# Jaroan/Contracts-MARL-AAM-Corridors

Measured on AMD Instinct MI355X. Metric: env-steps/sec (whole node) at 4096 envs x 10 agents, navigation_graph, higher is better.
Workload: dtype f64

## Files before the change

### contracts-marl-aam-corridors_amd/csrc/gmpe_kernel.h

```cpp
#pragma once
#include <hip/hip_runtime.h>
#include <math.h>
#include <stdio.h>
#include <stdlib.h>
#include <string.h>

#include <string>
#include <utility>
#include <vector>

#include "gmpe_device.h"

namespace gmpe {

enum { MODE_STEP = 0, MODE_RESET = 1 };
enum { SC_NAV = 0, SC_NAV_WALLS = 1, SC_JULY = 2, SC_ROT = 3, SC_TWO = 4, SC_THREE = 5, SC_COUNT = 6 };
__host__ __device__ constexpr bool sc_kinematic(int sc) { return sc >= SC_JULY; }
__host__ __device__ constexpr bool sc_rotfam(int sc) { return sc >= SC_ROT; }
__host__ __device__ constexpr bool sc_phasefam(int sc) { return sc == SC_TWO || sc == SC_THREE; }

struct KParams {
    gmpe_config c;
    DevState s;
    gmpe_outputs o;
// ... 107 lines not shown
template <int SC>
__device__ __forceinline__ void vel_of(double a2, double a3, double& vx, double& vy) {
    if (sc_kinematic(SC)) { double sn, cs; sincos(a2, &sn, &cs); vx = a3 * cs; vy = a3 * sn; }
    else { vx = a2; vy = a3; }
}

__device__ __forceinline__ bool wall_band_hit(const KParams& p, double px, double py, double size) {
    for (int w = 0; w < p.c.num_walls; ++w) {
        const gmpe_wall& wl = p.c.walls[w];
        const double band = 1.5 * size;
        const double perp = wl.orient == 0 ? py : px, prll = wl.orient == 0 ? px : py;
        if (wl.axis_pos - band <= perp && perp <= wl.axis_pos + band && wl.end0 - band <= prll && prll <= wl.end1 + band)
            return true;
    }
    return false;
}
__device__ __forceinline__ bool obstacle_collision_ego(const KParams& p, const Lds& l, int i) {
    const double* row = l.Dm + (size_t)i * p.E + p.A + p.L;
    for (int o = 0; o < p.O; ++o)
        if (row[o] < 2.0 * (p.c.entity_size + p.c.entity_size)) return true;
    return wall_band_hit(p, l.ex[i], l.ey[i], p.c.entity_size);
}

template <int SC>
__device__ __forceinline__ void decode_action(const gmpe_config& c, int idx, double& u0, double& u1) {
    if (!sc_kinematic(SC)) {
        if (c.n_actions == 5) {
            u0 = (idx == 1 ? 1.0 : 0.0) - (idx == 2 ? 1.0 : 0.0);
            u1 = (idx == 3 ? 1.0 : 0.0) - (idx == 4 ? 1.0 : 0.0);
        } else {
            const double d = 0.71;
            u0 = (idx == 1 ? -1.0 : idx == 5 ? 1.0 : (idx == 2 || idx == 8) ? -d : (idx == 4 || idx == 6) ? d : 0.0);
            u1 = (idx == 3 ? -1.0 : idx == 7 ? 1.0 : (idx == 2 || idx == 4) ? -d : (idx == 6 || idx == 8) ? d : 0.0);
        }
    } else {
        const int wi = idx / 5, ai = idx - wi * 5;
        u0 = wi == 0 ? c.ang_rate_opt[0] : wi == 1 ? c.ang_rate_opt[1] : wi == 2 ? c.ang_rate_opt[2] : wi == 3 ? c.ang_rate_opt[3] : c.ang_rate_opt[4];
        u1 = ai == 0 ? c.accel_opt[0] : ai == 1 ? c.accel_opt[1] : ai == 2 ? c.accel_opt[2] : ai == 3 ? c.accel_opt[3] : c.accel_opt[4];
    }
    u0 *= c.sensitivity; u1 *= c.sensitivity;
}

template <int AP, int SC>
__device__ __forceinline__ void write_obs(const KParams& p, const Lds& l, int i, double vx, double vy, int phase) {
    float* o = l.obs + (size_t)i * ((AP > 0 && (SC == SC_NAV || SC == SC_JULY)) ? (SC == SC_JULY ? 19 : 13) : p.D);
    const double px = l.ex[i], py = l.ey[i];
    const double gx = l.ex[(AP ? AP : p.A) + i] - px, gy = l.ey[(AP ? AP : p.A) + i] - py;
    o[0] = (float)px; o[1] = (float)py; o[2] = (float)vx; o[3] = (float)vy;
    o[4] = (float)gx; o[5] = (float)gy; o[6] = 0.0f; o[7] = (float)gx; o[8] = (float)gy;
    const double INF = __builtin_huge_val();
    int b1 = -1, b2 = -1; double d1 = INF, d2 = INF;
    const double* row = l.Dm + (size_t)i * ((AP > 0 && (SC == SC_NAV || SC == SC_JULY)) ? 2 * AP : p.E);
    if (AP) {
        double rv[AP ? AP : 1];
#pragma unroll
        for (int k = 0; k < AP; ++k) rv[k] = row[k < (AP ? AP : p.A) ? k : 0];
        __builtin_amdgcn_sched_barrier(0);
#pragma unroll
        for (int k = 0; k < AP; ++k) {
            const double d = (k < (AP ? AP : p.A) && k != i) ? rv[k] : INF;
            const bool lt1 = d < d1, lt2 = d < d2;
            d2 = lt1 ? d1 : (lt2 ? d : d2); b2 = lt1 ? b1 : (lt2 ? k : b2);
            d1 = lt1 ? d : d1; b1 = lt1 ? k : b1;
        }
    } else {
        for (int k = 0; k < (AP ? AP : p.A); ++k) {
            const double d = k != i ? row[k] : INF;
            const bool lt1 = d < d1, lt2 = d < d2;
            d2 = lt1 ? d1 : (lt2 ? d : d2); b2 = lt1 ? b1 : (lt2 ? k : b2);
            d1 = lt1 ? d : d1; b1 = lt1 ? k : b1;
        }
    }
    o[9] = b1 >= 0 ? (float)(l.ex[b1] - px) : 0.f; o[10] = b1 >= 0 ? (float)(l.ey[b1] - py) : 0.f;
    o[11] = b2 >= 0 ? (float)(l.ex[b2] - px) : 0.f; o[12] = b2 >= 0 ? (float)(l.ey[b2] - py) : 0.f;
    if (SC == SC_JULY) {
        o[13] = (float)(l.tube[T_ENTX] - px); o[14] = (float)(l.tube[T_ENTY] - py);
        o[15] = (float)(l.tube[T_EXX] - px); o[16] = (float)(l.tube[T_EXY] - py);
        o[17] = (float)l.tube[T_WIDTH]; o[18] = (float)phase;
    }
}

template <int AP, int SC>
__device__ __forceinline__ void write_obs_rot(const KParams& p, const Lds& l, int i, int phase) {
    float* o = l.obs + (size_t)i * p.D;
    const double px = l.ex[i], py = l.ey[i], th = l.s2[i];
    double sn, cs; sincos(th, &sn, &cs);
    const double INF = __builtin_huge_val();
    int b1 = -1, b2 = -1; double d1 = INF, d2 = INF;
    const double* row = l.Dm + (size_t)i * p.E;
    for (int k = 0; k < p.A; ++k) {
        bool skip = k == i;
        if (sc_phasefam(SC)) skip = skip || l.s_old[k] || (l.newf[k] && k < i);
        const double d = !skip ? row[k] : INF;
        const bool lt1 = d < d1, lt2 = d < d2;
        d2 = lt1 ? d1 : (lt2 ? d : d2); b2 = lt1 ? b1 : (lt2 ? k : b2);
        d1 = lt1 ? d : d1; b1 = lt1 ? k : b1;
    }
    double gx, gy;
    if (SC == SC_TWO) rot2(cs, sn, (double)(float)l.tube[T_EXX] - px, (double)(float)l.tube[T_EXY] - py, gx, gy);
    else rot2(cs, sn, l.ex[p.A + i] - px, l.ey[p.A + i] - py, gx, gy);
    double n1x = 0, n1y = 0, n2x = 0, n2y = 0;
    if (b1 >= 0) rot2(cs, sn, (double)(float)(l.ex[b1] - px), (double)(float)(l.ey[b1] - py), n1x, n1y);
    if (b2 >= 0) rot2(cs, sn, (double)(float)(l.ex[b2] - px), (double)(float)(l.ey[b2] - py), n2x, n2y);
    const double L = l.tube[T_L], hw = l.tube[T_HALFW];
    double s, yy; tube_sy(l.tube, px, py, s, yy);
    o[0] = (float)cs; o[1] = (float)sn; o[2] = (float)l.s3[i];
    o[3] = (float)gx; o[4] = (float)gy; o[5] = (float)n1x; o[6] = (float)n1y; o[7] = (float)n2x; o[8] = (float)n2y;
    o[9] = (float)clipd(s / L, -2.0, 2.0); o[10] = (float)clipd(yy / (hw + 1e-9), -2.0, 2.0);
    o[11] = (float)(exit_gate_distance(s, yy, L, hw) / (L + 1e-9));
    if (sc_phasefam(SC)) {
        double hs, hc; sincos(heading_error_signed(l.tube, th), &hs, &hc);
        o[12] = (float)hc; o[13] = (float)hs; o[14] = (float)phase;
    } else o[12] = (float)phase;
}

__device__ __forceinline__ double win_draw(const KParams& p, double* buf, int64_t& base, int W, int n, int i, int64_t k, int& err) {
    if (k >= base + W) {
        base = k;
        const int64_t kk = k + i;
        double val;
        if (p.s.tape) val = kk < p.s.tape_len ? p.s.tape[(size_t)n * p.s.tape_len + kk] : __builtin_nan("");
        else val = philox_uniform(p.c.seed, (uint32_t)(p.c.env_id_base + n), (uint64_t)kk);
        __builtin_amdgcn_fence(__ATOMIC_ACQUIRE, "wavefront");
        buf[i] = val;
        __builtin_amdgcn_fence(__ATOMIC_RELEASE, "wavefront");
        __builtin_amdgcn_wave_barrier();
        __builtin_amdgcn_fence(__ATOMIC_ACQUIRE, "wavefront");
    }
    double v = buf[(int)(k - base)];
    if (v != v) { err |= 1; v = 0.5; }
    return v;
}

__device__ __forceinline__ bool closer_than(double dx, double dy, double thr) {
    const double d2 = dx * dx + dy * dy, t2 = thr * thr;
    if (d2 < t2 * (1.0 - 1e-12)) return true;
    if (d2 > t2 * (1.0 + 1e-12)) return false;
    return sqrt(d2) < thr;
}
__device__ __forceinline__ double draw_raw(const KParams& p, int n, int64_t k) {
    if (p.s.tape) return k < p.s.tape_len ? p.s.tape[(size_t)n * p.s.tape_len + k] : 0.5;
    return philox_uniform(p.c.seed, (uint32_t)(p.c.env_id_base + n), (uint64_t)k);
}
__device__ __forceinline__ void wave_lds_sync() {
    __builtin_amdgcn_fence(__ATOMIC_RELEASE, "wavefront");
    __builtin_amdgcn_wave_barrier();
    __builtin_amdgcn_fence(__ATOMIC_ACQUIRE, "wavefront");
}
struct DrawBuf { const double* d; int64_t base; int nd; };
__device__ __forceinline__ double buf_get(const KParams& p, const DrawBuf& w, int n, int64_t k) {
    const int64_t o = k - w.base;
    return o < w.nd ? w.d[o] : draw_raw(p, n, k);
}
__device__ __forceinline__ void place_uniform(const KParams& p, const Lds& l, const DrawBuf& win, int n, int i, bool mine, unsigned long long emask, int M, int base, double thr,
                                              bool check_static, bool is_agent, int64_t& ctr, int& err) {
    const gmpe_config& c = p.c;
    const int A = p.A, O = p.O, o0 = p.A + p.L;
    const double ws = c.world_size, size = c.entity_size, lo = -ws / 2, hi = ws / 2;
    const int lane0 = emask ? __ffsll((long long)emask) - 1 : 0;
    double* cx = l.vox; double* cy = l.voy;
    unsigned long long* cm = reinterpret_cast<unsigned long long*>(l.vnx);
    int k = 0, tries = 0;
    while (__ballot(mine && k < M)) {
        if (mine && k < M) {
            const double px = 0.8 * (lo + (hi - lo) * buf_get(p, win, n, ctr + 2 * i));
            const double py = 0.8 * (lo + (hi - lo) * buf_get(p, win, n, ctr + 2 * i + 1));
            bool bad0 = false;
            if (check_static) {
                bad0 = wall_band_hit(p, px, py, size);
                for (int o = 0; o < O; ++o) bad0 = bad0 || closer_than(l.ex[o0 + o] - px, l.ey[o0 + o] - py, 2.0 * (size + size));
            }
            for (int q = 0; q < k; ++q) bad0 = bad0 || closer_than(l.ex[base + q] - px, l.ey[base + q] - py, thr);
            cx[i] = px; cy[i] = py;
            wave_lds_sync();
            unsigned long long cl = 0ull;
            for (int j = 0; j < i; ++j) if (closer_than(cx[j] - px, cy[j] - py, thr)) cl |= 1ull << j;
            cm[i] = cl;
            wave_lds_sync();
            const unsigned long long bad = (__ballot(bad0) & emask) >> lane0;
            unsigned long long acc = 0ull;
            int kk = k, t = tries, used = 0, slot = -1;
            for (int j = 0; j < A && kk < M; ++j) {
                const bool b = ((bad >> j) & 1ull) || (cm[j] & acc) != 0ull;
                used = j + 1;
                if (b && ++t < GMPE_MAX_TRIES) continue;
                if (b) err |= 2;
                if (j == i) slot = kk;
                acc |= 1ull << j; ++kk; t = 0;
            }
            wave_lds_sync();
            if (slot >= 0) {
                l.ex[base + slot] = px; l.ey[base + slot] = py;
                if (is_agent) { l.n2[slot] = 0.0; l.n3[slot] = 0.0; }
            }
            wave_lds_sync();
            ctr += 2 * used; k = kk; tries = t;
        }
    }
}

template <int SC, bool BATCH = false>
__device__ __forceinline__ void reset_world_coop(const KParams& p, const Lds& l, int n, int i, bool mine, unsigned long long emask, int64_t& ctr, int& err) {
    const gmpe_config& c = p.c;
    const double ws = c.world_size, size = c.entity_size;
    const int A = p.A, L = p.L, O = p.O;
    const int o0 = A + L;
    int64_t wbase = -(int64_t)A - 1;
    const int64_t ctr_in = ctr;
    const DrawBuf win = {reinterpret_cast<const double*>(l.M), ctr, BATCH ? (p.E * p.E + 3) / 4 * 2 : 0};
    const int lane0 = emask ? __ffsll((long long)emask) - 1 : 0;
#define WDRAW(k) (BATCH ? buf_get(p, win, n, (k)) : win_draw(p, l.serr, wbase, A, n, i, (k), err))
    if (sc_kinematic(SC)) {
        double entx = 0, enty = 0, exx = 0, exy = 0, sa = 0, ca = 1;
        if (mine) {
            (void)WDRAW(ctr++);
            const double a = 3 * size * 2.5, b = ws * 0.15;
            const double width = a > b ? a : b;
            const double angle = -M_PI / 2 + (M_PI / 2 - (-M_PI / 2)) * WDRAW(ctr++);
            double tl = ws * 0.8;
            if (sc_phasefam(SC)) tl += -ws * 0.3 + (ws * 0.1 - (-ws * 0.3)) * WDRAW(ctr++);
            ca = cos(angle); sa = sin(angle);
            const double be = tl / 4, bx = -tl / 4;
            entx = ca * 0 + sa * be; enty = -sa * 0 + ca * be;
            exx = ca * 0 + sa * bx; exy = -sa * 0 + ca * bx;
            const double dx = exx - entx, dy = exy - enty;
            const double Lt = sqrt(dx * dx + dy * dy) + 1e-9;
            const double ex = dx / Lt, ey = dy / Lt;
            if (i == 0) {
                double* t = l.tube;
                t[T_ANGLE] = angle; t[T_ENTX] = entx; t[T_ENTY] = enty; t[T_EXX] = exx; t[T_EXY] = exy;
                t[T_EX] = ex; t[T_EY] = ey; t[T_NX] = (double)(float)(-ey); t[T_NY] = (double)(float)ex;
                t[T_L] = Lt; t[T_HALFW] = width * 0.5; t[T_WIDTH] = width;
                for (int q = 0; q < GMPE_TUBE_STRIDE; ++q) p.s.tube[(size_t)n * GMPE_TUBE_STRIDE + q] = t[q];
            }
        }
        int k = 0, tries = 0;
        double mx = 0, my = 0;
        if constexpr (BATCH) while (__ballot(mine && k < A)) {
            if (mine && k < A) {
                const double u0 = buf_get(p, win, n, ctr + 2 * i), u1 = buf_get(p, win, n, ctr + 2 * i + 1);
                constexpr bool rot = sc_rotfam(SC);
                const double jf = rot ? 0.3 : 0.2;
                const double jx = jf * (-ws + (ws - (-ws)) * u0), jy = jf * (-ws + (ws - (-ws)) * u1);
                const double dfe = rot ? (ws + k) / 3 : (ws + k) / 5;
                const double px = entx + dfe * sa + jx, py = enty + dfe * ca + jy;
                bool bad_i = wall_band_hit(p, px, py, size);
                for (int o = 0; o < O; ++o) bad_i = bad_i || closer_than(l.ex[o0 + o] - px, l.ey[o0 + o] - py, 2.0 * (size + size));
                for (int q = 0; q < k; ++q) bad_i = bad_i || closer_than(l.ex[q] - px, l.ey[q] - py, c.sep_dist);
                const unsigned long long all = emask >> lane0;
                const unsigned long long good = ~((__ballot(bad_i) & emask) >> lane0) & all;
                const int jg = good ? __ffsll((long long)good) - 1 : A;
                const int jfo = GMPE_MAX_TRIES - 1 - tries;
                int js;
                if (jfo < A && jfo < jg) { js = jfo; err |= 2; }
                else if (jg < A) js = jg;
                else { tries += A; ctr += 2 * A; continue; }
                ctr += 2 * (js + 1);
                const double th = 0.0 + (2 * M_PI - 0.0) * buf_get(p, win, n, ctr); ++ctr;
                if (i == js) { l.ex[k] = px; l.ey[k] = py; l.n2[k] = th; l.n3[k] = c.v_min; }
                wave_lds_sync();
                ++k; tries = 0;
            }
        }
        else while (__ballot(mine && k < A)) {
            if (mine && k < A) {
                const double u0 = WDRAW(ctr), u1 = WDRAW(ctr + 1);
                ctr += 2;
                constexpr bool rot = sc_rotfam(SC);
                const double jf = rot ? 0.3 : 0.2;
                const double jx = jf * (-ws + (ws - (-ws)) * u0), jy = jf * (-ws + (ws - (-ws)) * u1);
                const double dfe = rot ? (ws + k) / 3 : (ws + k) / 5;
                const double px = entx + dfe * sa + jx, py = enty + dfe * ca + jy;
                bool bad_i = wall_band_hit(p, px, py, size);
                for (int o = i; o < O; o += A) bad_i = bad_i || norm2(l.ex[o0 + o] - px, l.ey[o0 + o] - py) < 2.0 * (size + size);
                bad_i = bad_i || (i < k && norm2(mx - px, my - py) < c.sep_dist);
                const bool bad = (__ballot(bad_i) & emask) != 0ull;
                if (bad && ++tries < GMPE_MAX_TRIES) continue;
                if (bad) err |= 2;
                const double th = 0.0 + (2 * M_PI - 0.0) * WDRAW(ctr++);
                if (i == k) { mx = px; my = py; l.ex[k] = px; l.ey[k] = py; l.n2[k] = th; l.n3[k] = c.v_min; }
                ++k; tries = 0;
            }
        }
        if (mine) {
            if (c.formation_type == GMPE_FORMATION_LINE) {
                const int div = L - 1;
                const double s0 = -ws / 2, e0 = ws / 2, ddx = e0 - s0, ddy = s0 - s0;
                for (int q = i; q < L; q += A) {
                    const double f = div > 0 ? (double)q / (double)div : (double)q;
                    double lx = f * ddx + s0, ly = f * ddy + s0;
                    if (L > 1 && q == L - 1) { lx = e0; ly = s0; }
                    bool hit = wall_band_hit(p, lx, ly, size);
                    for (int o = 0; o < O; ++o) hit = hit || norm2(l.ex[o0 + o] - lx, l.ey[o0 + o] - ly) < 2.0 * (size + size);
                    if (hit) err |= 2;
                    l.ex[A + q] = lx; l.ey[A + q] = ly;
                }
            } else if (c.formation_type == GMPE_FORMATION_CIRCLE) {
                const double cy = exy + ws / 5, radius = ws / 3, angle_step = 2 * M_PI / L;
                for (int q = i; q < L; q += A) {
                    const double ang = q * angle_step;
                    l.ex[A + q] = 0.0 + radius * cos(ang); l.ey[A + q] = cy + radius * sin(ang);
                }
            } else {
                const double rel = -ws / 3;
                const double rx = ca * 0.0 + sa * rel, ry = -sa * 0.0 + ca * rel;
                for (int q = i; q < L; q += A) { l.ex[A + q] = exx + rx; l.ey[A + q] = exy + ry; }
            }
        }
    } else if constexpr (BATCH) {
        place_uniform(p, l, win, n, i, mine, emask, O, o0, 2.0 * (size + size), false, false, ctr, err);
        place_uniform(p, l, win, n, i, mine, emask, A, 0, c.sep_dist, true, true, ctr, err);
        place_uniform(p, l, win, n, i, mine, emask, L, A, c.sep_dist, true, false, ctr, err);
        if (mine) for (int o = i; o < O; o += A) {
            p.s.obstacles[((size_t)n * O + o) * 2] = l.ex[o0 + o];
            p.s.obstacles[((size_t)n * O + o) * 2 + 1] = l.ey[o0 + o];
        }
    } else {
        const double lo = -ws / 2, hi = ws / 2;
        int k = 0, tries = 0;
        while (__ballot(mine && k < O)) {
            if (mine && k < O) {
                const double px = 0.8 * (lo + (hi - lo) * WDRAW(ctr));
                const double py = 0.8 * (lo + (hi - lo) * WDRAW(ctr + 1));
                ctr += 2;
                bool bad_i = false;
                for (int q = i; q < k; q += A) bad_i = bad_i || norm2(l.ex[o0 + q] - px, l.ey[o0 + q] - py) < 2.0 * (size + size);
                const bool bad = (__ballot(bad_i) & emask) != 0ull;
                if (bad && ++tries < GMPE_MAX_TRIES) continue;
                if (bad) err |= 2;
                if (k % A == i) { l.ex[o0 + k] = px; l.ey[o0 + k] = py; }
                ++k; tries = 0;
            }
        }
        k = 0; tries = 0;
        double mx = 0, my = 0;
        while (__ballot(mine && k < A)) {
            if (mine && k < A) {
                const double px = 0.8 * (lo + (hi - lo) * WDRAW(ctr));
                const double py = 0.8 * (lo + (hi - lo) * WDRAW(ctr + 1));
                ctr += 2;
                bool bad_i = wall_band_hit(p, px, py, size);
                for (int o = i; o < O; o += A) bad_i = bad_i || norm2(l.ex[o0 + o] - px, l.ey[o0 + o] - py) < 2.0 * (size + size);
                bad_i = bad_i || (i < k && norm2(mx - px, my - py) < c.sep_dist);
                const bool bad = (__ballot(bad_i) & emask) != 0ull;
                if (bad && ++tries < GMPE_MAX_TRIES) continue;
                if (bad) err |= 2;
                if (i == k) { mx = px; my = py; l.ex[k] = px; l.ey[k] = py; l.n2[k] = 0.0; l.n3[k] = 0.0; }
                ++k; tries = 0;
            }
        }
        k = 0; tries = 0;
        while (__ballot(mine && k < L)) {
            if (mine && k < L) {
                const double px = 0.8 * (lo + (hi - lo) * WDRAW(ctr));
                const double py = 0.8 * (lo + (hi - lo) * WDRAW(ctr + 1));
                ctr += 2;
                bool bad_i = wall_band_hit(p, px, py, size);
                for (int o = i; o < O; o += A) bad_i = bad_i || norm2(l.ex[o0 + o] - px, l.ey[o0 + o] - py) < 2.0 * (size + size);
                for (int r = i; r < k; r += A) bad_i = bad_i || norm2(l.ex[A + r] - px, l.ey[A + r] - py) < c.sep_dist;
                const bool bad = (__ballot(bad_i) & emask) != 0ull;
                if (bad && ++tries < GMPE_MAX_TRIES) continue;
                if (bad) err |= 2;
                if (k % A == i) { l.ex[A + k] = px; l.ey[A + k] = py; }
                ++k; tries = 0;
            }
        }
        if (mine) for (int o = i; o < O; o += A) {
            p.s.obstacles[((size_t)n * O + o) * 2] = l.ex[o0 + o];
            p.s.obstacles[((size_t)n * O + o) * 2 + 1] = l.ey[o0 + o];
        }
    }
    if (mine) for (int q = i; q < L; q += A) {
        p.s.landmarks[((size_t)n * L + q) * 2] = l.ex[A + q];
        p.s.landmarks[((size_t)n * L + q) * 2 + 1] = l.ey[A + q];
    }
    if (BATCH && mine && p.s.tape && ctr > ctr_in && ctr > p.s.tape_len) err |= 1;
}
#undef WDRAW


template <int BLOCK, int U, int CA>
__device__ __forceinline__ void distance_trip(const KParams& p, const Lds& l, int q0, int total, int W, int dv, bool even, bool only_reset) {
    const int A = CA ? CA : p.A, E = CA ? 2 * CA : p.E, AE = A * E, EE4 = (E * E + 3) / 4 * 4;
    double ds[U]; int gs[U], rs[U], cs[U];
#pragma unroll
    for (int u = 0; u < U; ++u) {
        const int q = q0 + u * BLOCK;
        const bool live = q < total;
        const int qq = live ? q : 0;
        const int g = fdiv(qq, W, p.m_W), w = qq - g * W;
        const int a = fdiv(w, dv, p.m_Sx), b = w - a * dv;
        int r, cc;
        if (even) { const bool up = b >= a; r = up ? a : E - 1 - a; cc = up ? b + 1 : E - a + b; }
        else { int c0 = a + 1 + b; c0 = c0 >= E ? c0 - E : c0; r = a < c0 ? a : c0; cc = a < c0 ? c0 : a; }
        const double dx = l.ex[g * E + r] - l.ex[g * E + cc], dy = l.ey[g * E + r] - l.ey[g * E + cc];
        ds[u] = (GMPE_ABL(p) & 16) ? dx * dx + dy * dy : sqrt(dx * dx + dy * dy);
        gs[u] = (live && !(only_reset && !l.flags[g * 4 + 0])) ? g : -1; rs[u] = r; cs[u] = cc;
    }
#pragma unroll
    for (int u = 0; u < U; ++u) {
        if (gs[u] < 0) continue;
        const int r = rs[u], cc = cs[u];
        float* Mg = l.M + (size_t)gs[u] * EE4;
        const float df = (float)ds[u];
        Mg[r * E + cc] = df; Mg[cc * E + r] = df;
        if (r < A) {
            double* Dg = l.Dm + (size_t)gs[u] * AE;
            Dg[r * E + cc] = ds[u];
            if (cc < A) Dg[cc * E + r] = ds[u];
        }
    }
}
template <int BLOCK, int CA>
__device__ __forceinline__ void distance_pass(const KParams& p, const Lds& l, int G, int tid, bool only_reset) {
    const int A = CA ? CA : p.A, E = CA ? 2 * CA : p.E, AE = A * E, EE4 = (E * E + 3) / 4 * 4;
    const int W = E * (E - 1) / 2;
    const bool even = (E & 1) == 0;
    const int dv = even ? E - 1 : (E - 1) / 2;
    const int total = G * W;
    const int wave_base = tid & ~63;
    for (int base = 0; base + wave_base < total; base += 5 * BLOCK) {
        const int left = total - (base + wave_base);
        const int nu = (left + BLOCK - 1) / BLOCK;
        const int q0 = base + tid;
        if (nu >= 5) distance_trip<BLOCK, 5, CA>(p, l, q0, total, W, dv, even, only_reset);
        else if (nu == 4) distance_trip<BLOCK, 4, CA>(p, l, q0, total, W, dv, even, only_reset);
        else if (nu == 3) distance_trip<BLOCK, 3, CA>(p, l, q0, total, W, dv, even, only_reset);
        else if (nu == 2) distance_trip<BLOCK, 2, CA>(p, l, q0, total, W, dv, even, only_reset);
        else distance_trip<BLOCK, 1, CA>(p, l, q0, total, W, dv, even, only_reset);
    }
    for (int q = tid; q < G * E; q += BLOCK) {
        const int g = fdiv(q, E, p.m_E), r = q - g * E;
        if (only_reset && !l.flags[g * 4 + 0]) continue;
        l.M[(size_t)g * EE4 + r * E + r] = 0.0f;
        if (r < A) l.Dm[(size_t)g * AE + r * E + r] = 0.0;
    }
}

#define GMPE_NSTAMPS 32
#ifdef GMPE_STAMPS
#define STAMP(k) do { if (tid == 0 && p.stamps) p.stamps[(size_t)blockIdx.x * GMPE_NSTAMPS + (k)] = __builtin_readcyclecounter(); } while (0)
#define STAMP_T(k, t) do { if (tid == (t) && p.stamps) p.stamps[(size_t)blockIdx.x * GMPE_NSTAMPS + (k)] = __builtin_readcyclecounter(); } while (0)
#else
#define STAMP(k) do { } while (0)
#define STAMP_T(k, t) do { } while (0)
#endif
template <int BLOCK, int CA, bool FORCES>
__device__ __forceinline__ void distance_force_pass(const KParams& p, const Lds& l, int G, int Gv, int tid, bool only_reset, bool statics) {
    constexpr int A = CA, E = 2 * CA, AE = A * E, EE4 = (E * E + 3) / 4 * 4, NP = A * (A - 1) / 2, NL = A * A;
    const gmpe_config& c = p.c;
    double* Fx = l.F2; double* Fy = Fx + (size_t)G * A * A;
    const int n1 = Gv * NP, n2 = n1 + Gv * NL, total = n2 + (statics ? Gv * NP : 0);
    const int wave_base = tid & ~63;
    for (int base = 0; base + wave_base < total; base += 3 * BLOCK) {
        double ds[3], dxs[3], dys[3]; int gs[3], rs[3], cs[3];
#pragma unroll
        for (int u = 0; u < 3; ++u) {
            const int q = base + u * BLOCK + tid;
            const bool live = q < total;
            const int qq = live ? q : 0;
            int g, r, cc;
            if (qq < n1) { g = qq / NP; const int pk = l.ptab[qq - g * NP]; r = pk >> 8; cc = pk & 255; }
            else if (qq < n2) { const int t = qq - n1; g = t / NL; const int w = t - g * NL; r = w / A; cc = A + (w - r * A); }
            else { const int t = qq - n2; g = t / NP; const int pk = l.ptab[t - g * NP]; r = A + (pk >> 8); cc = A + (pk & 255); }
            const double dx = l.ex[g * E + r] - l.ex[g * E + cc], dy = l.ey[g * E + r] - l.ey[g * E + cc];
            dxs[u] = dx; dys[u] = dy; ds[u] = sqrt(dx * dx + dy * dy);
            gs[u] = (live && !(only_reset && !l.flags[g * 4 + 0])) ? g : -1; rs[u] = r; cs[u] = cc;
        }
#pragma unroll
        for (int u = 0; u < 3; ++u) {
            if (gs[u] < 0) continue;
            const int r = rs[u], cc = cs[u];
            float* Mg = l.M + (size_t)gs[u] * EE4;
            const float df = (float)ds[u];
            Mg[r * E + cc] = df; Mg[cc * E + r] = df;
            if (r < A) {
                double* Dg = l.Dm + (size_t)gs[u] * AE;
                Dg[r * E + cc] = ds[u];
                if (cc < A) Dg[cc * E + r] = ds[u];
            }
        }
#pragma unroll
        for (int u = 0; u < 3; ++u) {
            if (!FORCES) break;
            if (base + u * BLOCK + wave_base >= n1) continue;
            if (gs[u] < 0 || cs[u] >= A) continue;
            const double dmin = c.contact_family ? c.agent_size + c.agent_size : c.sep_dist;
            const double pen = logaddexp0(-(ds[u] - dmin) / c.contact_margin) * c.contact_margin;
            const int slot = gs[u] * A * A + rs[u] * A + cs[u];
            Fx[slot] = c.contact_force * dxs[u] / ds[u] * pen; Fy[slot] = c.contact_force * dys[u] / ds[u] * pen;
        }
    }
    for (int q = tid; q < G * E; q += BLOCK) {
        const int g = q / E, r = q - g * E;
        if (only_reset && !l.flags[g * 4 + 0]) continue;
        if (r >= A && !statics) continue;
        l.M[(size_t)g * EE4 + r * E + r] = 0.0f;
        if (r < A) l.Dm[(size_t)g * AE + r * E + r] = 0.0;
    }
}

#define SWEEP(var, n) _Pragma("unroll") for (int var = 0; var < (AP ? AP : (n)); ++var)
template <int BLOCK, int AP, int SC, int FL>
__device__ __forceinline__ void stream_graph_fn(const KParams& p, const gmpe_outputs& o, const Lds& l, const int Gv, const int n0, const int tid,
                                                const int t0, const int nthr, const bool do_mask, const int any_mask) {
    constexpr bool CT = AP > 0 && SC != SC_NAV_WALLS;
    const int A = CT ? AP : p.A, L = CT ? AP : p.L, E = CT ? 2 * AP : p.E, EE = E * E, EE4 = (EE + 3) / 4 * 4;
    const int abl = FL ? 0 : GMPE_ABL(p);
    const bool nt = FL == 1 ? false : p.nt != 0;
    if (do_mask && any_mask && !(abl & 4)) {
        for (int q = tid; q < Gv * EE; q += BLOCK) {
            const int gg = fdiv(q, EE, p.m_EE), rc = q - gg * EE;
            if (!l.flags[gg * 4 + 2]) continue;
            const int r = fdiv(rc, E, p.m_E), cc = rc - r * E;
            if (l.moff[gg * E + r] | l.moff[gg * E + cc]) l.M[(size_t)gg * EE4 + rc] = 0.0f;
        }
    }
    if (do_mask) __syncthreads();
    

    if (o.adj && !(abl & 1)) {
        const bool vec = (EE & 3) == 0;
        if (o.adj_compact) {
            float* dst = o.adj + (size_t)n0 * EE;
            if (vec) {
                const int nq = EE / 4;
                for (int q = t0; q < Gv * nq; q += nthr) {
                    const int gg = fdiv(q, nq, p.m_nq), m = q - gg * nq;
                    if (l.flags[gg * 4 + 3]) reinterpret_cast<float4*>(dst)[q] = reinterpret_cast<const float4*>(l.M + (size_t)gg * EE4)[m];
                }
            } else for (int q = t0; q < Gv * EE; q += nthr) { const int gg = fdiv(q, EE, p.m_EE); if (l.flags[gg * 4 + 3]) dst[q] = l.M[(size_t)gg * EE4 + (q - gg * EE)]; }
        } else {
            float* dst = o.adj + (size_t)n0 * A * EE;
#ifdef GMPE_NTORDER_KNOB
            if (vec && nt && p.ablate != 200) {
#else
            if (vec && nt) {
#endif
                const int nq = EE / 4, per = A * nq;
                for (int gg = 0; gg < Gv; ++gg) {
                    if (!l.flags[gg * 4 + 3]) continue;
                    const float4* M4 = reinterpret_cast<const float4*>(l.M + (size_t)gg * EE4);
                    float4* d4 = reinterpret_cast<float4*>(dst) + (size_t)gg * per;
                    for (int q = t0; q < per; q += nthr) {
                        const int a = fdiv(q, nq, p.m_nq), m = q - a * nq;
                        nt_store4(&d4[q], M4[m]);
                    }
                }
            } else if (vec) {
                const int nq = EE / 4;
                for (int q = t0; q < Gv * nq; q += nthr) {
                    const int gg = fdiv(q, nq, p.m_nq), m = q - gg * nq;
                    if (!l.flags[gg * 4 + 3]) continue;
                    const float4 val = reinterpret_cast<const float4*>(l.M + (size_t)gg * EE4)[m];
                    float4* d4 = reinterpret_cast<float4*>(dst) + (size_t)gg * A * nq + m;
                    SWEEP(a, A) { if (!AP || a < A) { if (nt) nt_store4(&d4[(size_t)a * nq], val); else d4[(size_t)a * nq] = val; } }
                }
            } else {
                const int AEE = A * EE;
                for (int q = t0; q < Gv * AEE; q += nthr) {
                    const int gg = q / AEE, rem = q - gg * AEE, rc = rem % EE;
                    if (l.flags[gg * 4 + 3]) dst[q] = l.M[(size_t)gg * EE4 + rc];
                }
            }
        }
    }
    
    STAMP_T(16, 64); STAMP_T(19, 192);
    if (o.entity_table) {
        const int W = p.TW;
        double* dst = o.entity_table + (size_t)n0 * W;
        for (int q = t0; q < Gv * W; q += nthr) {
            const int gg = fdiv(q, W, p.m_TW), w = q - gg * W;
            if (!l.flags[gg * 4 + 3]) continue;
            double val;
            const int wm = W - (E + 31) / 32;
            if (w < 2 * E) val = w < E ? l.ex[gg * E + w] : l.ey[gg * E + (w - E)];
            else if (w >= wm) {
                unsigned bits = 0;
                const int k0 = (w - wm) * 32;
                for (int b = 0; b < 32 && k0 + b < E; ++b) bits |= (l.moff[gg * E + k0 + b] ? 1u : 0u) << b;
                val = (double)bits;
            }
            else if (SC == SC_TWO && w >= wm - 2) val = l.tube[gg * GMPE_TUBE_STRIDE + (w == wm - 2 ? T_EXX : T_EXY)];
            else {
                const int r = w - 2 * E, blk = fdiv(r, A, p.m_A), a = gg * A + (r - blk * A);
                val = blk == 0 ? l.vox[a] : blk == 1 ? l.voy[a] : blk == 2 ? l.vnx[a] : blk == 3 ? l.vny[a] : blk == 4 ? l.cn[a] : l.sn[a];
            }
            dst[q] = val;
        }
    }
    if (sc_rotfam(SC) && o.node_obs && !(abl & 2) && p.c.graph_feat_type != 1) {
// ... 541 lines not shown
                            double hx, hy; sincos(v.s2[i], &hy, &hx);
                            int front = -1, back = -1; double fproj = 0, bproj = 0;
                            for (int k = 0; k < A; ++k) {
                                if (k == i) continue;
                                const double pj = (v.ex[k] - px) * hx + (v.ey[k] - py) * hy;
                                if (pj > 0) { if (front < 0 || pj < fproj) { front = k; fproj = pj; } }
                                else { if (back < 0 || pj > bproj) { back = k; bproj = pj; } }
                            }
                            if (front >= 0) { const double df = row[front] - c.sep_dist; serr += df < 0 ? fabs(df) : 0; }
                            if (back >= 0) { const double df = row[back] - c.sep_dist; serr += df < 0 ? fabs(df) : 0; }
                            if (serr > 0) sv += 1;
                            rew -= serr * c.formation_rew;
                            rew -= exit_gate_distance(ts, ty, Lt, hw);
                            if (rotinv) {
                                const double tdx = v.tube[T_EXX] - v.tube[T_ENTX], tdy = v.tube[T_EXY] - v.tube[T_ENTY];
                                const double tlen = sqrt(tdx * tdx + tdy * tdy);
                                const double proj = (px - v.tube[T_ENTX]) * (tdx / tlen) + (py - v.tube[T_ENTY]) * (tdy / tlen);
                                const double gain = c.goal_rew / (c.world_size * 0.8 * 10);
                                const double dproj = proj - pproj;
                                rew += gain * (dproj > -0.05 ? dproj : -0.05);
                                pproj = (double)(float)proj;
                            } else rew -= herr * c.formation_rew * 0.1;
                            sic += 1;
                        } else if (rotinv && cp == 2 && phase_reached == 0) cp = 0;
                        else if (cp == 2 && !two) {
                            if (dgoal < c.goal_thresh) { if (me_new) rew += c.goal_rew * 5; }
                            else rew -= dgoal;
                        }
                        if (phase_reached == 1 && cp == 0) conf += 1;
                        if (cp > phase_reached) phase_reached = cp;
                        if (cp < prev_phase) rew -= c.collision_rew;
                        if (cp < phase_reached) rew -= c.collision_rew;
                        prev_phase = cp;
                        if (in_tube_rect(ts, ty, Lt, hw) && cp != 1 && !(three && in_exit_gate(ts, ty, Lt, hw, 0.02))) rew -= c.collision_rew;
                        if (ts > Lt && phase_reached < 1) rew -= c.goal_rew;
                    } else {
                        if (dgoal < c.goal_thresh) { if (me_new) rew += c.goal_rew * 5; }
                        else rew -= dgoal;
                    }
                    rew = clipd(rew, -4 * c.collision_rew, c.goal_rew * 5);
                    if (!rotfam) rew = clipd(rew, c.min_reward, c.max_reward);
                    v.serr[i] = two ? 0.0 : serr; v.rew[i] = rew;

                    STAMP(15);
                    v.dtg_o[i] = dtg; v.trq_o[i] = trq;
                    int nearest = 0; double dmin = INF;
                    SWEEP(q, L) { const bool ok = !AP || q < L; const double d = ok ? row[A + (ok ? q : 0)] : INF; const bool lt = d < dmin; dmin = lt ? d : dmin; nearest = lt ? q : nearest; }
                    const double thr = c.goal_thresh;
                    const int tnow = (int)((double)cur_step * c.dt);
                    if (dmin < thr && (nearest != greached && greached != -1)) { greached = nearest; dleft = (int)dmin; }
                    if (dmin < thr && trq == -1) { trq = tnow; dtg = (int)p_dist; dleft = (int)dmin; greached = nearest; }
                    if (trq == -1) { dtg = (int)p_dist; dleft = (int)dmin; }
                    if (dmin > thr && trq != -1) { dtg = (int)p_dist; trq = tnow; dleft = (int)dmin; }
                    if (dmin < thr && nearest == greached) { dleft = (int)dmin; greached = nearest; }
                    v.dtg_n[i] = dtg; v.trq_n[i] = trq;
                    v.sv_n[i] = sv; v.sv_o[i] = sv - (serr > 0 ? 1 : 0);
                }
                if (block_sync) __syncthreads();
                else {
                    __builtin_amdgcn_fence(__ATOMIC_RELEASE, "wavefront");
                    __builtin_amdgcn_wave_barrier();
                    __builtin_amdgcn_fence(__ATOMIC_ACQUIRE, "wavefront");
                }
                STAMP(6);

                if (ag) {
                    double rsum = 0;
                    if (c.collaborative) for (int a = 0; a < A; ++a) rsum += v.rew[a];
                    if (out.reward) out.reward[na] = (float)(c.collaborative ? rsum : rew);
                    if (out.done) out.done[na] = done ? 1 : 0;
                    if (ROLL) {
                        if (p.masks) p.masks[(size_t)slot * p.st_mask + na] = done ? 0.0f : 1.0f;
                        if (p.active) p.active[(size_t)slot * p.st_mask + na] = (done && !all_done) ? 0.0f : 1.0f;
                    }
                    if (out.info) {
                        double sd = 0, st = 0, sdd = 0, stt = 0; int ssv = 0;
                        SWEEP(a, A) {
                            const bool ok = !AP || a < A;
                            const int ac = ok ? a : 0;
                            const bool nw = ac <= i;
                            const int dn = v.dtg_n[ac], d_o = v.dtg_o[ac], tn = v.trq_n[ac], to = v.trq_o[ac], svn = v.sv_n[ac], svo = v.sv_o[ac];
                            const double dd = ok ? (double)(nw ? dn : d_o) : 0.0, tt = ok ? (double)(nw ? tn : to) : 0.0;
                            sd += dd; st += tt; sdd += dd * dd; stt += tt * tt;
                            ssv += ok ? (nw ? svn : svo) : 0;
                        }
                        double dsp = dsp0;
                        if (july || rotfam) for (int a = 0; a <= i; ++a) dsp += v.serr[a];
                        const double dm = sd / A, tm = st / A;
                        const double dvn = (double)A * sdd - sd * sd, tvn = (double)A * stt - st * st;
                        const double ds = sqrt(dvn) / A, ts = sqrt(tvn) / A;
                        float* o = out.info + na * GMPE_INFO_KEYS;
                        o[0] = (float)rew; o[1] = (float)dleft; o[2] = (float)trq; o[3] = (float)nac; o[4] = (float)noc;
                        o[5] = (float)dm; o[6] = (float)ds; o[7] = (float)(dm / (ds + 0.0001)); o[8] = (float)dtg;
                        o[9] = (float)trq; o[10] = (float)tm; o[11] = (float)ts; o[12] = (float)(tm / (ts + 0.0001));
                        o[13] = (float)((double)conf / c.episode_length);
                        o[14] = (float)(dsp / (ssv != 0 ? (double)ssv : 1.0));
                        o[15] = (float)((double)sv / (sic != 0 ? sic : 1));
                        o[16] = (float)gmt;
                        o[17] = (float)phase_reached;
                    }
                    if (ROLL && !all_done && kk + 1 < K) {
                        int* ci = l.cnt + (size_t)(g * A + i) * 9;
                        ci[0] = trq; ci[1] = dtg; ci[2] = dleft; ci[3] = greached; ci[4] = nac; ci[5] = noc; ci[6] = sv; ci[7] = sic; ci[8] = conf;
                        if (rotinv) l.cntd[(size_t)(g * A + i) * 2 + 1] = pproj;
                        if (i == 0) {
                            double dsp = dsp0;
                            if (july || rotfam) for (int a = 0; a < A; ++a) dsp += v.serr[a];
                            l.cntd[(size_t)G * A * 2 + g] = dsp;
                        }
                    } else if (!all_done) {
                        if (i == 0) {
                            double dsp = dsp0;
                            if (july || rotfam) for (int a = 0; a < A; ++a) dsp += v.serr[a];
                            p.s.delta_spacing[n] = dsp;
                            p.s.rng_ctr[n] = ctr0 + v.flags[1];
                            p.s.current_step[n] = cur_step;
                        }
                        p.s.x[na] = v.ex[i]; p.s.y[na] = v.ey[i]; p.s.s2[na] = v.n2[i]; p.s.s3[na] = v.n3[i];
                        p.s.status[na] = (uint8_t)(v.s_old[i] || v.newf[i]);
                        p.s.prev_phase[na] = prev_phase; p.s.phase_reached[na] = phase_reached; p.s.cooldown[na] = cooldown;
                        p.s.goal_tracker[na] = v.gt[i]; p.s.p_dist[na] = p_dist; p.s.time[na] = tim;
                        p.s.times_required[na] = trq; p.s.dists_to_goal[na] = dtg; p.s.dist_left[na] = dleft;
                        p.s.goal_reached[na] = greached; p.s.n_agent_coll[na] = nac; p.s.n_obst_coll[na] = noc;
                        p.s.spacing_viol[na] = sv; p.s.steps_in_corr[na] = sic; p.s.conformance[na] = conf;
                        if (rotinv) p.s.prev_proj[na] = pproj;
                    }
                }
                STAMP(7);
                if (spec && !ROLL) {
                    __builtin_amdgcn_fence(__ATOMIC_RELEASE, "wavefront");
                    __builtin_amdgcn_wave_barrier();
                    __builtin_amdgcn_fence(__ATOMIC_ACQUIRE, "wavefront");
                    if (out.obs) {
                        float* dst = out.obs + (size_t)n0 * A * D;
                        const int AD = A * D;
                        for (int q = tid; q < Gv * AD; q += 64) { const int gg = fdiv(q, AD, p.m_AD); if (l.flags[gg * 4 + 3]) dst[q] = l.obs[(size_t)gg * AD4 + (q - gg * AD)]; }
                    }
                    if (out.agent_id) for (int q = tid; q < Gv * A; q += 64) { const int gg = fdiv(q, A, p.m_A); if (l.flags[gg * 4 + 3]) out.agent_id[(size_t)n0 * A + q] = q - gg * A; }
                }
            }
            else {
                STAMP_T(9, 64); STAMP_T(17, 192);
                stream_graph_fn<BLOCK, AP, SC, FL>(p, out, l, Gv, n0, tid, tid - 64, BLOCK - 64, false, any_mask);
                STAMP_T(10, 64); STAMP_T(18, 192);
            }
            __syncthreads();
        }
        {
            if (any_reset) {
                const bool mine = ag && v.flags[0];
                if (tid < 64) {
                    int64_t ctr = ctr0 + ((mine && step) ? v.flags[1] : 0);
                    STAMP(20);
                    reset_world_coop<SC, BATCHK>(p, v, n, i, mine, emask, ctr, err);
                    STAMP(21);
                    if (mine && i == 0) {
                        if (ROLL) reinterpret_cast<long long*>(l.cntd + (size_t)G * A * 2 + G)[g] = ctr;
                        p.s.rng_ctr[n] = ctr;
                        p.s.current_step[n] = 0;
                        p.s.delta_spacing[n] = 0.0;
                        v.flags[2] = 0;
                    }
                }
                __syncthreads();
                if (mine) {
                    v.s2[i] = v.n2[i]; v.s3[i] = v.n3[i];
                    double vx, vy; vel_of<SC>(v.n2[i], v.n3[i], vx, vy);
                    v.vox[i] = v.vnx[i] = vx; v.voy[i] = v.vny[i] = vy;
                    v.s_old[i] = 0; v.newf[i] = 0; v.gt[i] = -1; v.moff[i] = 0; v.moff[A + i] = 0;
                    int prevA = prev_phase, ph = 0;
                    if (july) ph = phase_eval(v.tube, v.ex[i], v.ey[i], prev_phase, prevA);
                    prev_phase = prevA;
                    if (rotfam) { ph = phase_eval_rot<PV>(v.tube, v.ex[i], v.ey[i], prev_phase, 0); double sn_, cn_; sincos(v.n2[i], &sn_, &cn_); v.cn[i] = cn_; v.sn[i] = sn_; p.s.prev_proj[na] = 0.0; }
                    const double dx = v.ex[i] - v.ex[A + i], dy = v.ey[i] - v.ey[A + i];
                    gmt = c.max_speed > 0 ? sqrt(dx * dx + dy * dy) / c.max_speed : 0.0;
                    p.s.x[na] = v.ex[i]; p.s.y[na] = v.ey[i]; p.s.s2[na] = v.n2[i]; p.s.s3[na] = v.n3[i];
                    p.s.status[na] = 0; p.s.prev_phase[na] = prev_phase; p.s.phase_reached[na] = 0; p.s.cooldown[na] = 0;
                    p.s.goal_tracker[na] = -1; p.s.p_dist[na] = 0.0; p.s.time[na] = 0.0;
                    p.s.times_required[na] = -1; p.s.dists_to_goal[na] = -1; p.s.dist_left[na] = -1;
                    p.s.goal_reached[na] = -1; p.s.n_agent_coll[na] = 0; p.s.n_obst_coll[na] = 0;
                    p.s.spacing_viol[na] = 0; p.s.steps_in_corr[na] = 0; p.s.conformance[na] = 0;
                    p.s.goal_min_time[na] = gmt;
                    ph1 = ph;
                }
                STAMP(22);
                __syncthreads();
                if constexpr (FUSE_OK) {
                    if (FUSE) distance_force_pass<BLOCK, AP, !kin>(p, l, G, Gv, tid, true, true);
                    else distance_pass<BLOCK, (CT ? AP : 0)>(p, l, Gv, tid, true);
                } else distance_pass<BLOCK, (CT ? AP : 0)>(p, l, Gv, tid, true);
                __syncthreads();
                STAMP(23);
                if (mine) { if (rotfam) write_obs_rot<AP, SC>(p, v, i, ph1); else write_obs<AP, SC>(p, v, i, v.vox[i], v.voy[i], ph1); }
                any_mask = 0;
                for (int gg = 0; gg < Gv; ++gg) any_mask |= l.flags[gg * 4 + 2];
            }
            STAMP(8);
        }
        if (ROLL && !early) {
            __builtin_amdgcn_fence(__ATOMIC_RELEASE, "workgroup");
            __syncthreads();
        }
        if (!early) stream_graph_fn<BLOCK, AP, SC, FL>(p, out, l, Gv, n0, tid, tid, BLOCK, true, any_mask);
        STAMP(11);
        if (!spec || ROLL) {
            if (out.obs) {
                float* dst = out.obs + (size_t)n0 * A * D;
                const int AD = A * D;
                for (int q = tid; q < Gv * AD; q += BLOCK) { const int gg = fdiv(q, AD, p.m_AD); if (l.flags[gg * 4 + 3]) dst[q] = l.obs[(size_t)gg * AD4 + (q - gg * AD)]; }
            }
            if (out.agent_id) for (int q = tid; q < Gv * A; q += BLOCK) { const int gg = fdiv(q, A, p.m_A); if (l.flags[gg * 4 + 3]) out.agent_id[(size_t)n0 * A + q] = q - gg * A; }
        }
        if (ROLL && kk + 1 < K) {
            if (!early) __builtin_amdgcn_fence(__ATOMIC_RELEASE, "workgroup");
            if (!spec || !early) __syncthreads();
            if (ag) {
                if (all_done) {
                    phase_reached = 0; cooldown = 0; p_dist = 0.0; tim = 0.0; cur_step = 0;
                    ctr0 = reinterpret_cast<const long long*>(l.cntd + (size_t)G * A * 2 + G)[g];
                    int* ci = l.cnt + (size_t)(g * A + i) * 9;
                    ci[0] = -1; ci[1] = -1; ci[2] = -1; ci[3] = -1; ci[4] = 0; ci[5] = 0; ci[6] = 0; ci[7] = 0; ci[8] = 0;
                    l.cntd[(size_t)(g * A + i) * 2] = gmt; l.cntd[(size_t)(g * A + i) * 2 + 1] = 0.0;
                    if (i == 0) l.cntd[(size_t)G * A * 2 + g] = 0.0;
                } else {
                    v.s2[i] = v.n2[i]; v.s3[i] = v.n3[i];
                    v.s_old[i] = (v.s_old[i] || v.newf[i]) ? 1 : 0;
                    ctr0 += ndraw;
                }
                const int na_ = c.n_actions;
                act_idx = act_next < 0 ? 0 : (act_next >= na_ ? na_ - 1 : act_next);
            }
            for (int q = tid; q < G * E; q += BLOCK) l.moff[q] = 0;
            if (tid < G) {
                const bool active = n0 + tid < p.env_hi;
                l.flags[tid * 4 + 0] = 0; l.flags[tid * 4 + 1] = 0; l.flags[tid * 4 + 2] = 0; l.flags[tid * 4 + 3] = active;
            }
            slot = slot + 1 == p.num_slots ? 0 : slot + 1;
            __syncthreads();
        }
    } while (ROLL && ++kk < K);
    if (ag && err) atomicOr(&p.s.error_flags[n], err);
    STAMP(12);
}


struct EnvKernel {
    const void* fn;
    int threads;
    bool fuse;
};
template <int SC> EnvKernel env_kernel(int block, int ap, int fl, int G);

}
```

Baseline: 212.0 million.

## Specialize batched reset placement with compile-time agent count and unrolled masks

Adds a compile-time-size path for uniform placement during batched resets. It keeps the candidate-rejection loop in registers with unrolled squared-distance masks and a branchless greedy acceptance scan, and ping-pongs two LDS buffers to drop one wave barrier per round. It also assumes obstacles are zero and landmarks equal the agent count, and shrinks the draw window to match. The aim is to cut reset latency in the navigation scenario. The risk is divergence from the generic path if those assumptions do not hold, plus extra register pressure.

```diff
diff --git a/contracts-marl-aam-corridors_amd/csrc/gmpe_kernel.h b/contracts-marl-aam-corridors_amd/csrc/gmpe_kernel.h
--- a/contracts-marl-aam-corridors_amd/csrc/gmpe_kernel.h
+++ b/contracts-marl-aam-corridors_amd/csrc/gmpe_kernel.h
@@ -283,12 +283,111 @@
     const int64_t o = k - w.base;
     return o < w.nd ? w.d[o] : draw_raw(p, n, k);
 }
+#define GMPE_NSTAMPS 32
+#ifdef GMPE_STAMPS
+#define PSTAMP(k, val) do { if (threadIdx.x == 0 && p.stamps) p.stamps[(size_t)blockIdx.x * GMPE_NSTAMPS + (k)] = (val); } while (0)
+#else
+#define PSTAMP(k, val) do { } while (0)
+#endif
+template <int CA = 0>
 __device__ __forceinline__ void place_uniform(const KParams& p, const Lds& l, const DrawBuf& win, int n, int i, bool mine, unsigned long long emask, int M, int base, double thr,
                                               bool check_static, bool is_agent, int64_t& ctr, int& err) {
     const gmpe_config& c = p.c;
     const int A = p.A, O = p.O, o0 = p.A + p.L;
     const double ws = c.world_size, size = c.entity_size, lo = -ws / 2, hi = ws / 2;
     const int lane0 = emask ? __ffsll((long long)emask) - 1 : 0;
+    if constexpr (CA > 0) {
+        static_assert(CA <= 16, "a sweep's mask is half of a 32-bit word");
+        constexpr int N1 = CA > 1 ? CA : 1;
+        const int row = (int)(l.s3 - l.s2);
+        const double* ex = l.ex + base; const double* ey = l.ey + base;
+        const double t2 = thr * thr, t2lo = t2 * (1.0 - 1e-12), t2hi = t2 * (1.0 + 1e-12);
+        int k = 0, tries = 0, set = 0, rounds = 0;
+        while (__ballot(mine && k < CA)) {
+            if (mine && k < CA) {
+                if (is_agent && k == 0) PSTAMP(24, __builtin_readcyclecounter());
+                const int so = set ? row : 0;
+                double* cx = l.s2 + so; double* cy = l.vox + so; unsigned* cm = reinterpret_cast<unsigned*>(l.vnx + so);
+                const int64_t o = ctr + 2 * i - win.base;
+                double u0 = 0.0, u1 = 0.0;
+                if (o + 1 < win.nd) { u0 = win.d[o]; u1 = win.d[o + 1]; }
+                else {
+#pragma unroll 1
+                    for (int d = 0; d < 2; ++d) { u0 = u1; u1 = draw_raw(p, n, ctr + 2 * i + d); }
+                }
+                const double px = 0.8 * (lo + (hi - lo) * u0), py = 0.8 * (lo + (hi - lo) * u1);
+                cx[i] = px; cy[i] = py;
+                wave_lds_sync();
+                unsigned ltm = 0u, ngm = 0u;
+                {
+                    double qx[N1], qy[N1];
+#pragma unroll
+                    for (int q = 0; q < CA; ++q) { qx[q] = ex[q]; qy[q] = ey[q]; }
+                    __builtin_amdgcn_sched_barrier(0);
+#pragma unroll
+                    for (int q = 0; q < CA; ++q) {
+                        const double dx = qx[q] - px, dy = qy[q] - py, d2 = dx * dx + dy * dy;
+                        ltm |= d2 < t2lo ? 1u << q : 0u;
+                        ngm |= !(d2 > t2hi) ? 1u << q : 0u;
+                    }
+                }
+                const unsigned km = (1u << k) - 1u, im = (1u << i) - 1u;
+                unsigned hit = ltm & km, band = ngm & ~ltm & km;
+                ltm = 0u; ngm = 0u;
+                {
+                    double jx[N1], jy[N1];
+#pragma unroll
+                    for (int j = 0; j < CA; ++j) { jx[j] = cx[j]; jy[j] = cy[j]; }
+                    __builtin_amdgcn_sched_barrier(0);
+#pragma unroll
+                    for (int j = 0; j < CA; ++j) {
+                        const double dx = jx[j] - px, dy = jy[j] - py, d2 = dx * dx + dy * dy;
+                        ltm |= d2 < t2lo ? 1u << j : 0u;
+                        ngm |= !(d2 > t2hi) ? 1u << j : 0u;
+                    }
+                }
+                unsigned cl = ltm & im;
+                band |= (ngm & ~ltm & im) << 16;
+                while (band) {
+                    const int b = __ffs((int)band) - 1, q = b & 15; band &= band - 1u;
+                    if (closer_than((b < 16 ? ex : cx)[q] - px, (b < 16 ? ey : cy)[q] - py, thr)) { if (b < 16) hit |= 1u << q; else cl |= 1u << q; }
+                }
+                const bool bad0 = hit != 0u;
+                cm[i] = cl;
+                wave_lds_sync();
+                const unsigned bad = (unsigned)((__ballot(bad0) & emask) >> lane0);
+                unsigned cmr[N1];
+#pragma unroll
+                for (int j = 0; j < CA; ++j) cmr[j] = cm[j];
+                __builtin_amdgcn_sched_barrier(0);
+                unsigned acc = 0u;
+                int kk = k, t = tries, used = 0;
+#pragma unroll
+                for (int j = 0; j < CA; ++j) {
+                    const unsigned live = (unsigned)(kk - CA) >> 31;
+                    const unsigned b = ((bad >> j) & 1u) | min(cmr[j] & acc, 1u);
+                    const unsigned forced = b & ((unsigned)(GMPE_MAX_TRIES - 2 - t) >> 31);
+                    const unsigned take = live & ((b ^ 1u) | forced);
+                    used += (int)live;
+                    err |= (int)((live & forced) << 1);
+                    t = (t + (int)live) & ((int)take - 1);
+                    acc |= take << j;
+                    kk += (int)take;
+                }
+                const int slot = ((acc >> i) & 1u) ? k + __popc(acc & ((1u << i) - 1u)) : -1;
+                if (slot >= 0) {
+                    l.ex[base + slot] = px; l.ey[base + slot] = py;
+                    if (is_agent) { l.n2[slot] = 0.0; l.n3[slot] = 0.0; }
+                }
+                if (is_agent && k == 0) PSTAMP(25, __builtin_readcyclecounter());
+                ctr += 2 * used; k = kk; tries = t; set ^= 1;
+            }
+            ++rounds;
+        }
+        wave_lds_sync();
+        PSTAMP(is_agent ? 26 : 27, (unsigned long long)rounds);
+        return;
+    }
     double* cx = l.vox; double* cy = l.voy;
     unsigned long long* cm = reinterpret_cast<unsigned long long*>(l.vnx);
     int k = 0, tries = 0;
@@ -330,7 +429,7 @@
     }
 }
 
-template <int SC, bool BATCH = false>
+template <int SC, bool BATCH = false, int CA = 0>
 __device__ __forceinline__ void reset_world_coop(const KParams& p, const Lds& l, int n, int i, bool mine, unsigned long long emask, int64_t& ctr, int& err) {
     const gmpe_config& c = p.c;
     const double ws = c.world_size, size = c.entity_size;
@@ -338,7 +437,7 @@
     const int o0 = A + L;
     int64_t wbase = -(int64_t)A - 1;
     const int64_t ctr_in = ctr;
-    const DrawBuf win = {reinterpret_cast<const double*>(l.M), ctr, BATCH ? (p.E * p.E + 3) / 4 * 2 : 0};
+    const DrawBuf win = {reinterpret_cast<const double*>(l.M), ctr, BATCH ? ((CA ? 4 * CA * CA : p.E * p.E) + 3) / 4 * 2 : 0};
     const int lane0 = emask ? __ffsll((long long)emask) - 1 : 0;
 #define WDRAW(k) (BATCH ? buf_get(p, win, n, (k)) : win_draw(p, l.serr, wbase, A, n, i, (k), err))
     if (sc_kinematic(SC)) {
@@ -438,6 +537,10 @@
                 for (int q = i; q < L; q += A) { l.ex[A + q] = exx + rx; l.ey[A + q] = exy + ry; }
             }
         }
+    } else if constexpr (BATCH && CA > 0) {
+#pragma unroll 1
+        for (int cls = 0; cls < 2; ++cls)
+            place_uniform<CA>(p, l, win, n, i, mine, emask, CA, cls * CA, c.sep_dist, true, cls == 0, ctr, err);
     } else if constexpr (BATCH) {
         place_uniform(p, l, win, n, i, mine, emask, O, o0, 2.0 * (size + size), false, false, ctr, err);
         place_uniform(p, l, win, n, i, mine, emask, A, 0, c.sep_dist, true, true, ctr, err);
@@ -568,7 +671,6 @@
     }
 }
 
-#define GMPE_NSTAMPS 32
 #ifdef GMPE_STAMPS
 #define STAMP(k) do { if (tid == 0 && p.stamps) p.stamps[(size_t)blockIdx.x * GMPE_NSTAMPS + (k)] = __builtin_readcyclecounter(); } while (0)
 #define STAMP_T(k, t) do { if (tid == (t) && p.stamps) p.stamps[(size_t)blockIdx.x * GMPE_NSTAMPS + (k)] = __builtin_readcyclecounter(); } while (0)
@@ -1416,7 +1518,7 @@
                 if (tid < 64) {
                     int64_t ctr = ctr0 + ((mine && step) ? v.flags[1] : 0);
                     STAMP(20);
-                    reset_world_coop<SC, BATCHK>(p, v, n, i, mine, emask, ctr, err);
+                    reset_world_coop<SC, BATCHK, (BATCHK ? AP : 0)>(p, v, n, i, mine, emask, ctr, err);
                     STAMP(21);
                     if (mine && i == 0) {
                         if (ROLL) reinterpret_cast<long long*>(l.cntd + (size_t)G * A * 2 + G)[g] = ctr;
```

Result: slower. 209.5 million (-1.2%).
